# kausaltech/reina-model

Measured on NVIDIA B200. Metric: agent-days/sec (HUS 1.7M), higher is better.
Workload: dtype int32/f32 state, f64 uniforms

## Files before the change

### include/reina_b200.h

```cpp
#ifndef REINA_B200_H
#define REINA_B200_H

#include <stdint.h>

#ifdef __cplusplus
extern "C" {
#endif

#define RB_MAX_AGES 128
#define RB_MAX_VARIANTS 4
#define RB_MAX_ROWS 96
#define RB_NCDF 100
#define RB_MAX_IMPORT_EVENTS 8
#define RB_MAX_VACC 8
#define RB_MAX_IMPORT_CLASSES 16
#define RB_N_PLACES 6
#define RB_IOT_LEN 21

enum { RB_ASYMPTOMATIC = 0, RB_MILD, RB_SEVERE, RB_CRITICAL, RB_FATAL };
enum { RB_SUSCEPTIBLE = 0, RB_INCUBATION, RB_ILLNESS, RB_HOSPITALIZED, RB_IN_ICU, RB_RECOVERED, RB_DEAD };
enum { RB_NO_PROBLEMOS = 0, RB_TOO_MANY_INFECTEES, RB_TOO_MANY_CONTACTS, RB_HOSPITAL_ACCOUNTING_FAILURE,
       RB_NEGATIVE_CONTACTS, RB_MALLOC_FAILURE, RB_OTHER_FAILURE, RB_WRONG_STATE,
       RB_CONTACT_PROBABILITY_FAILURE, RB_INFECTEES_MISMATCH };
enum { RB_NO_TESTING = 0, RB_ALL_WITH_SYMPTOMS_CT, RB_ALL_WITH_SYMPTOMS, RB_ONLY_SEVERE_SYMPTOMS };
// ... 72 lines not shown
int rb_create(const rb_config *cfg, const int32_t *age_counts, const int32_t *group_of_age,
              const rb_variant *variants, const int32_t *import_lo, const int32_t *import_hi,
              const float *import_cum, rb_engine **out);
void rb_destroy(rb_engine *e);

int rb_reset(rb_engine *e, uint32_t seed);

int rb_set_initial_state(rb_engine *e, const int32_t *ipc7);

int rb_set_contact_table(rb_engine *e, int32_t epoch, const int32_t *n_rows, const double *cum_p,
                         const int32_t *age_lo, const int32_t *age_hi, const uint8_t *place,
                         const float *mask_p, const double *nr_contacts, const double *ncontact_cdf);

int rb_set_schedule(rb_engine *e, int32_t day0, int32_t n, const rb_day_params *params);

int rb_step(rb_engine *e, int32_t n_days);
int rb_sync(rb_engine *e);
int32_t rb_day(rb_engine *e);

int rb_snapshot(rb_engine *e);
int32_t rb_row_len(rb_engine *e);
int rb_read_stats(rb_engine *e, int32_t day0, int32_t n, int32_t *out);

int rb_read_moments(rb_engine *e, int32_t day0, int32_t n, double *sum, double *sumsq);

int rb_read_per_age(rb_engine *e, int32_t replica, int32_t attr, int32_t *out);

int rb_problem(rb_engine *e, int32_t *out);

int rb_sample(rb_engine *e, int32_t what, int32_t age, int32_t severity, int32_t n, int32_t *out);

int rb_rng_block(int32_t words, uint32_t key, const uint32_t *ctr, uint32_t *out);

int rb_read_agents(rb_engine *e, int32_t replica, rb_agent *out);
int rb_read_queue(rb_engine *e, int32_t replica, int32_t *out, int32_t cap, int32_t *n);
int rb_read_available(rb_engine *e, int32_t replica, int32_t *beds_icu);
float rb_last_step_ms(rb_engine *e);
#define RB_N_KERNELS 5
int rb_step_profiled(rb_engine *e, int32_t n_days, float *ms_per_kernel);
int rb_step_timed(rb_engine *e, int32_t n_days, float *ms_per_kernel, int32_t *launches_per_kernel, float *wall_ms);
int rb_comm_init(rb_engine *e, int32_t rank, int32_t nranks, const uint8_t *unique_id128);
int32_t rb_comm_rank(rb_engine *e);
int32_t rb_comm_size(rb_engine *e);
int rb_comm_allreduce(rb_engine *e, double *inout, int64_t n, int32_t op);
int rb_comm_allgather(rb_engine *e, const void *in, void *out, int64_t bytes_per_rank);
int rb_reduce_moments(rb_engine *e, int32_t day0, int32_t n, double *sum, double *sumsq, int64_t *n_replicas);

int rb_shard_unique_id(uint8_t *out128);
int rb_shard_init(rb_engine *e, int32_t rank, int32_t nranks, const uint8_t *unique_id128, float exchange_capacity);
int rb_shard_init_local(rb_engine **engines, int32_t nranks, float exchange_capacity);
int32_t rb_shard_rank(rb_engine *e);
int32_t rb_shard_nranks(rb_engine *e);
int64_t rb_shard_message_bytes(rb_engine *e);
int32_t rb_shard_exchange(rb_engine *e);

int64_t rb_state_bytes(rb_engine *e);
int rb_save_state(rb_engine *e, void *out, int64_t capacity);
int rb_load_state(rb_engine *e, const void *in, int64_t n_bytes);

void rb_debug_flag(rb_engine *e, int32_t flag);
int rb_debug_phase_cycles(rb_engine *e, int32_t replica, long long *out16);

int64_t rb_launch_count(rb_engine *e);
int64_t rb_copied_bytes(rb_engine *e, int32_t direction);
const char *rb_last_error(void);

// ... 5 lines not shown
```

### reina_b200/_abi.py

```python
import ctypes as C
import os

import numpy as np

RB_MAX_AGES = 128
RB_MAX_VARIANTS = 4
RB_MAX_ROWS = 96
RB_NCDF = 100
RB_MAX_IMPORT_EVENTS = 8
RB_MAX_VACC = 8
RB_MAX_IMPORT_CLASSES = 16
RB_N_PLACES = 6
RB_IOT_LEN = 21
RB_N_TABLES = 6

ATTRS = ['susceptible', 'vaccinated', 'infected', 'all_infected', 'detected', 'all_detected',
         'in_icu', 'cum_icu', 'in_ward', 'dead', 'recovered', 'non_hospital_deaths', 'new_infections']
RB_N_ATTRS = len(ATTRS)
SCALARS = ['available_icu_units', 'available_hospital_beds', 'total_icu_units', 'total_hospital_beds',
           'total_infections', 'total_infectors', 'exposed_per_day', 'ct_cases_per_day', 'table_epoch',
           'day']
RB_S_CONTACTS0 = len(SCALARS)
RB_S_VARIANT0 = RB_S_CONTACTS0 + RB_N_PLACES
RB_N_SCALARS = RB_S_VARIANT0 + RB_MAX_VARIANTS
# ... 27 lines not shown


class DayParams(C.Structure):
    _fields_ = [
        ('testing_mode', C.c_int32), ('p_detected_anyway', C.c_float),
        ('p_successful_tracing', C.c_float), ('beds_delta', C.c_int32), ('icu_delta', C.c_int32),
        ('table_epoch', C.c_int32), ('n_imports', C.c_int32),
        ('import_amount', C.c_int32 * RB_MAX_IMPORT_EVENTS),
        ('import_variant', C.c_int32 * RB_MAX_IMPORT_EVENTS),
        ('trickle', C.c_int32 * RB_MAX_VARIANTS), ('n_vacc', C.c_int32),
        ('vacc_nr', C.c_int32 * RB_MAX_VACC), ('vacc_min_age', C.c_int32 * RB_MAX_VACC),
        ('vacc_max_age', C.c_int32 * RB_MAX_VACC), ('vacc_slot', C.c_int32 * RB_MAX_VACC),
        ('import_traced', C.c_int32), ('reserved', C.c_int32 * 3),
    ]


AGENT_DTYPE = np.dtype([
    ('infector', '<i4'), ('n_infected', '<i4'), ('days_left', '<i2'), ('day_of_illness', '<i2'),
    ('day_of_vaccination', '<i2'), ('state', 'u1'), ('severity', 'u1'), ('variant', 'u1'),
    ('flags', 'u1'), ('ward_days', 'u1'), ('icu_days', 'u1')], align=True)
assert AGENT_DTYPE.itemsize == 20, AGENT_DTYPE.itemsize

_HERE = os.path.dirname(os.path.abspath(__file__))
CUDA_LIB_PATH = os.environ.get('REINA_B200_LIB') or os.path.join(_HERE, 'libreina_b200.so')

SYMBOLS = ['create', 'destroy', 'reset', 'set_initial_state', 'step_profiled', 'set_contact_table', 'set_schedule', 'step', 'sync', 'day',
           'snapshot', 'row_len', 'read_stats', 'read_moments', 'read_per_age', 'problem', 'sample', 'read_agents',
           'read_queue', 'read_available', 'last_step_ms', 'launch_count', 'last_error', 'rng_block']


SHARD_SYMBOLS = ['shard_unique_id', 'shard_init', 'shard_init_local', 'shard_rank', 'shard_nranks', 'shard_message_bytes', 'shard_exchange',
                 'state_bytes', 'save_state', 'load_state',
                 'comm_init', 'comm_rank', 'comm_size', 'comm_allreduce', 'comm_allgather', 'reduce_moments',
                 'step_timed', 'debug_flag', 'debug_phase_cycles', 'copied_bytes']
SH_SHIFT = 12


def owner_of(agent_index, nranks):
    return (np.asarray(agent_index) >> SH_SHIFT) % nranks


class EngineError(RuntimeError):
    pass


def _ptr(a, ctype):
    return a.ctypes.data_as(C.POINTER(ctype))


class Library:

    def __init__(self, path, prefix):
        if not os.path.exists(path):
            raise EngineError(
                '%s not found: build it with `python -c "import __graft_entry__ as g; g.build()"` '
                '(there is no CPU fallback)' % path)
        self.path, self.prefix = path, prefix
        self.dll = C.CDLL(path)
        f = {}
        for name in SYMBOLS:
            f[name] = getattr(self.dll, prefix + name)
        vp = C.c_void_p
        f['create'].argtypes = [C.POINTER(Config), C.POINTER(C.c_int32), C.POINTER(C.c_int32),
                                C.POINTER(Variant), C.POINTER(C.c_int32), C.POINTER(C.c_int32),
                                C.POINTER(C.c_float), C.POINTER(vp)]
        f['destroy'].argtypes = [vp]
        f['destroy'].restype = None
# ... 24 lines not shown
        f['last_step_ms'].argtypes = [vp]
        f['last_step_ms'].restype = C.c_float
        f['launch_count'].argtypes = [vp]
        f['launch_count'].restype = C.c_int64
        f['last_error'].argtypes = []
        f['last_error'].restype = C.c_char_p
        if prefix == 'rb_':
            for name in SHARD_SYMBOLS:
                f[name] = getattr(self.dll, prefix + name)
            f['shard_unique_id'].argtypes = [C.c_char_p]
            f['shard_init'].argtypes = [vp, C.c_int32, C.c_int32, C.c_char_p, C.c_float]
            f['shard_init_local'].argtypes = [C.POINTER(vp), C.c_int32, C.c_float]
            f['shard_rank'].argtypes = [vp]
            f['shard_nranks'].argtypes = [vp]
            f['shard_message_bytes'].argtypes = [vp]
            f['shard_message_bytes'].restype = C.c_int64
            f['shard_exchange'].argtypes = [vp]
            f['state_bytes'].argtypes = [vp]
            f['state_bytes'].restype = C.c_int64
            f['save_state'].argtypes = [vp, C.c_void_p, C.c_int64]
            f['load_state'].argtypes = [vp, C.c_void_p, C.c_int64]
            f['comm_init'].argtypes = [vp, C.c_int32, C.c_int32, C.c_char_p]
            f['comm_rank'].argtypes = [vp]
            f['comm_size'].argtypes = [vp]
            f['comm_allreduce'].argtypes = [vp, C.POINTER(C.c_double), C.c_int64, C.c_int32]
            f['comm_allgather'].argtypes = [vp, C.c_void_p, C.c_void_p, C.c_int64]
            f['reduce_moments'].argtypes = [vp, C.c_int32, C.c_int32, C.POINTER(C.c_double), C.POINTER(C.c_double), C.POINTER(C.c_int64)]
            f['step_timed'].argtypes = [vp, C.c_int32, C.POINTER(C.c_float), C.POINTER(C.c_int32), C.POINTER(C.c_float)]
            f['debug_flag'].argtypes = [vp, C.c_int32]
            f['debug_flag'].restype = None
            f['debug_phase_cycles'].argtypes = [vp, C.c_int32, C.c_void_p]
            f['copied_bytes'].argtypes = [vp, C.c_int32]
            f['copied_bytes'].restype = C.c_int64
        self.f = f

    def check(self, rc, what):
        if rc != 0:
            raise EngineError('%s%s failed (%d): %s' % (
                self.prefix, what, rc, (self.f['last_error']() or b'').decode(errors='replace')))


_cuda_lib = None


def cuda_library():
    global _cuda_lib
    if _cuda_lib is None:
        _cuda_lib = Library(CUDA_LIB_PATH, 'rb_')
    return _cuda_lib


class Engine:

    def __init__(self, lib, cfg, age_counts, group_of_age, variants, import_lo, import_hi, import_cum):
        self.lib = lib
        self.cfg = cfg
        self.n_agents, self.n_ages = cfg.n_agents, cfg.n_ages
        self.n_groups, self.n_replicas = cfg.n_groups, cfg.n_replicas
        age_counts = np.ascontiguousarray(age_counts, dtype=np.int32)
        group_of_age = np.ascontiguousarray(group_of_age, dtype=np.int32)
        import_lo = np.ascontiguousarray(import_lo, dtype=np.int32)
        import_hi = np.ascontiguousarray(import_hi, dtype=np.int32)
        import_cum = np.ascontiguousarray(import_cum, dtype=np.float32)
        varr = (Variant * len(variants))(*variants)
        h = C.c_void_p()
        lib.check(lib.f['create'](C.byref(cfg), _ptr(age_counts, C.c_int32), _ptr(group_of_age, C.c_int32),
# ... 183 lines not shown
```

### reina_b200/csrc/engine.cu

```cuda
#include "state.cuh"
#include "boundary.cuh"
#include "sweep.cuh"
#include "contacts.cuh"
#include "shard.cuh"
#include "setup.cuh"
#include "run.cuh"

static thread_local char g_err[512];
#define CK(call) do { cudaError_t e_ = (call); if (e_ != cudaSuccess) { snprintf(g_err, sizeof g_err, "%s:%d %s: %s", __FILE__, __LINE__, #call, cudaGetErrorString(e_)); return 1; } } while (0)

#define MAX_GROUPS 8
struct ReplicaGroup {
    int r0, R;
    int sweep_blocks, list_blocks, resolve_blocks;
    cudaStream_t stream;
    cudaEvent_t ev_stagger, ev_join;
    cudaGraphExec_t graph[2];
};

struct rb_engine {
    rb_config cfg;
    Eng G;
    cudaStream_t stream;
    cudaEvent_t ev0, ev1;
    std::vector<void *> allocs;
    std::vector<DevTable *> tables;
    std::vector<std::vector<uint8_t>> table_args, table_host;
    DevTable **d_tables;
    int n_table_slots;
    rb_day_params *d_sched;
    double *d_moments;
    void *h_stage; int n_stage;
    cudaEvent_t ev_stage[4];
    std::vector<rb_day_params> h_sched;
    std::vector<int32_t> age_start, age_counts;
    std::vector<rb_variant> h_variants;
    int32_t day;
    float last_ms;
    int64_t launches;
    int64_t h2d_bytes, d2h_bytes;
    int sweep_blocks, list_blocks, resolve_blocks;
    cudaGraphExec_t graph[2];
    bool have_graphs;
    cudaError_t launch_err;
// ... 146 lines not shown
    float cc = cfg->contact_capacity > 0 ? cfg->contact_capacity : 1.0f;
    G.cap_items = pow2_at_least((uint64_t)((double)N * cc) + 4096);
    G.cap_succ = pow2_at_least((uint64_t)N / 8 + 4096);
    G.cap_events = pow2_at_least((uint64_t)N / 16 + 2048);
    G.cap_queue = pow2_at_least((uint64_t)N / 8 + 2048);
    const size_t RN = (size_t)R * G.Npad;
    cudaDeviceProp prop; CK(cudaGetDeviceProperties(&prop, cfg->device));
    const int sms = prop.multiProcessorCount;
    e->run_ctas = 0; e->run_boundary_ctas = 1;
    {
        int per_sm = 0;
        CK(cudaOccupancyMaxActiveBlocksPerMultiprocessor(&per_sm, k_run, RUN_THREADS, 0));
        const long long total = (long long)per_sm * sms;
        bool on = false;
        if (const char *s = getenv("RB_PERSISTENT")) on = atoi(s) != 0;
        if (on && total >= 2LL * R) {
            long long t = total / R; if (t > 64) t = 64;
            if (const char *s = getenv("RB_RUN_CTAS")) { const int v = atoi(s); if (v >= 1 && (long long)v * R <= total) t = v; }
            e->run_ctas = (int)t;
            int b = 1; while (b * 2 <= t && b * 2 <= 16) b *= 2;
            e->run_boundary_ctas = b;
        }
    }
    {
        int ng, pct;
        group_config(R, &ng, &pct);
        long long ctas = (long long)sms * SW_CTAS_PER_SM * (ng > 1 ? pct : 100) / 100 / ((R + ng - 1) / ng);
        if (ctas < 1) ctas = 1;
        long long S = 2 * ctas * SW_WARPS, most = (long long)N / 256;
        if (e->run_ctas) S = 2LL * e->run_ctas * RUN_WARPS;
        if (S > most) S = most;
        G.n_seg = (uint32_t)(S < 1 ? 1 : S);
        G.seg_cap = ((uint32_t)N + G.n_seg - 1) / G.n_seg;
    }
    G.sus_words = ((G.Npad + 31) / 32 + 32 + 3) & ~3;
    if (dalloc(e, &G.hot, RN) || dalloc(e, &G.perm, RN) || dalloc(e, &G.rec, RN) ||
        dalloc(e, &G.sus, (size_t)R * G.sus_words) || dalloc(e, &G.det, (size_t)R * G.sus_words) || dalloc(e, &G.alist, (size_t)R * 2 * G.n_seg * G.seg_cap) || dalloc(e, &G.seg_n, (size_t)R * 2 * G.n_seg) || dalloc(e, &G.items, (size_t)R * G.cap_items) || dalloc(e, &G.succ, (size_t)R * G.cap_succ) ||
        dalloc(e, &G.ev_key, (size_t)R * G.cap_events) || dalloc(e, &G.ev_agent, (size_t)R * G.cap_events) ||
        dalloc(e, &G.q_key, (size_t)R * 2 * G.cap_queue) || dalloc(e, &G.q_agent, (size_t)R * 2 * G.cap_queue) ||
        dalloc(e, &G.ctr, (size_t)R) || dalloc(e, &G.stats, (size_t)R * (cfg->max_days + 1) * G.row_len) ||
        dalloc(e, &e->d_sched, (size_t)cfg->max_days + 1) ||
        dalloc(e, &e->d_moments, 2 * ((size_t)cfg->max_days + 1) * G.row_len + 2)) { rb_destroy(e); return 1; }
    G.sched = e->d_sched;
    e->h_sched.assign(cfg->max_days + 1, rb_day_params());
    e->n_table_slots = 1024;
    if (dalloc(e, &e->d_tables, (size_t)e->n_table_slots)) { rb_destroy(e); return 1; }
    CK(cudaMemset(e->d_tables, 0, sizeof(DevTable *) * e->n_table_slots));
    G.tables = e->d_tables;
    e->tables.assign(e->n_table_slots, nullptr);
    rb_variant *dv; int32_t *d_as, *d_ga, *d_ilo, *d_ihi; float *d_icum; uint8_t *d_ab;
    if (dalloc(e, &dv, (size_t)cfg->n_variants) || dalloc(e, &d_as, (size_t)cfg->n_ages + 1) || dalloc(e, &d_ga, (size_t)cfg->n_ages) ||
        dalloc(e, &d_ilo, (size_t)RB_MAX_IMPORT_CLASSES) || dalloc(e, &d_ihi, (size_t)RB_MAX_IMPORT_CLASSES) ||
        dalloc(e, &d_icum, (size_t)RB_MAX_IMPORT_CLASSES) || dalloc(e, &d_ab, (size_t)(G.Npad >> 10) + 2)) { rb_destroy(e); return 1; }
    {
        std::vector<uint8_t> ab((size_t)(G.Npad >> 10) + 2);
        int age = 0;
        for (size_t b = 0; b < ab.size(); b++) {
            int64_t a = (int64_t)b << 10; if (a > N - 1) a = N - 1;
            while (age < cfg->n_ages - 1 && e->age_start[age + 1] <= a) age++;
            ab[b] = (uint8_t)age;
        }
        CK(cudaMemcpy(d_ab, ab.data(), ab.size(), cudaMemcpyHostToDevice));
    }
    e->h_variants.assign(variants, variants + cfg->n_variants);
    CK(cudaMemcpy(dv, variants, sizeof(rb_variant) * cfg->n_variants, cudaMemcpyHostToDevice));
    CK(cudaMemcpy(d_as, e->age_start.data(), sizeof(int32_t) * (cfg->n_ages + 1), cudaMemcpyHostToDevice));
    CK(cudaMemcpy(d_ga, group_of_age, sizeof(int32_t) * cfg->n_ages, cudaMemcpyHostToDevice));
    CK(cudaMemcpy(d_ilo, import_lo, sizeof(int32_t) * cfg->n_import_classes, cudaMemcpyHostToDevice));
    CK(cudaMemcpy(d_ihi, import_hi, sizeof(int32_t) * cfg->n_import_classes, cudaMemcpyHostToDevice));
    CK(cudaMemcpy(d_icum, import_cum, sizeof(float) * cfg->n_import_classes, cudaMemcpyHostToDevice));
    G.age_blk = d_ab; G.variants = dv; G.age_start = d_as; G.group_of_age = d_ga; G.import_lo = d_ilo; G.import_hi = d_ihi; G.import_cum = d_icum;
    e->age_counts.assign(age_counts, age_counts + cfg->n_ages);
    CK(cudaMemset(G.stats, 0, sizeof(int32_t) * (size_t)R * (cfg->max_days + 1) * G.row_len));
    CK(cudaMemset(e->d_sched, 0, sizeof(rb_day_params) * ((size_t)cfg->max_days + 1)));
    int want = ((int)G.n_seg + SW_WARPS - 1) / SW_WARPS;
// ... 690 lines not shown
    e->day += n_days;
    return 0;
}

extern "C" int rb_sync(rb_engine *e) {
    CK(cudaSetDevice(e->cfg.device));
    CK(cudaStreamSynchronize(e->stream));
    float ms = 0;
    if (cudaEventElapsedTime(&ms, e->ev0, e->ev1) == cudaSuccess) e->last_ms = ms; else cudaGetLastError();
    if (!e->shard_events.empty()) {
        double t[6] = {0, 0, 0, 0, 0, 0};
        for (size_t d = 0; d + 7 <= e->shard_events.size(); d += 7)
            for (int k = 0; k < 6; k++) { float x = 0; if (cudaEventElapsedTime(&x, e->shard_events[d + k], e->shard_events[d + k + 1]) == cudaSuccess) t[k] += x; }
        fprintf(stderr, "[rank %d] %zu days: sweep %.2f  expose %.2f  exchange+wait %.2f  merge %.2f  resolve %.2f  boundary %.2f ms (step %.2f)\n",
                e->G.rank, e->shard_events.size() / 7, t[0], t[1], t[2], t[3], t[4], t[5], e->last_ms);
        for (cudaEvent_t ev : e->shard_events) cudaEventDestroy(ev);
        e->shard_events.clear();
    }
    return 0;
}

extern "C" int32_t rb_day(rb_engine *e) { return e->day; }
extern "C" void rb_debug_flag(rb_engine *e, int32_t v) { e->G.dbg = v; }
extern "C" int rb_debug_phase_cycles(rb_engine *e, int32_t replica, long long *out16) {
    cudaSetDevice(e->cfg.device); cudaStreamSynchronize(e->stream);
    RepCtr c; if (cudaMemcpy(&c, &e->G.ctr[replica], sizeof c, cudaMemcpyDeviceToHost) != cudaSuccess) return 1;
    memcpy(out16, c.dbg_t, sizeof c.dbg_t); return 0;
}
extern "C" int rb_rng_block(int32_t words, uint32_t key, const uint32_t *ctr, uint32_t *out) {
    if (words == 4) { const u32x4 x = philox(key, ctr[0], ctr[1], ctr[2], ctr[3]); out[0] = x.x; out[1] = x.y; out[2] = x.z; out[3] = x.w; return 0; }
    snprintf(g_err, sizeof g_err, "rb_rng_block: words must be 4");
    return 1;
}
extern "C" int32_t rb_row_len(rb_engine *e) { return e->G.row_len; }
extern "C" float rb_last_step_ms(rb_engine *e) { return e->last_ms; }
extern "C" int64_t rb_launch_count(rb_engine *e) { return e->launches; }
extern "C" int64_t rb_copied_bytes(rb_engine *e, int32_t direction) { return direction == 0 ? e->h2d_bytes : e->d2h_bytes; }

extern "C" int rb_snapshot(rb_engine *e) {
    CK(cudaSetDevice(e->cfg.device));
    k_snapshot<<<e->G.R, 256, 0, e->stream>>>(e->G); e->launches++;
    CK(cudaGetLastError());
    return 0;
}

extern "C" int rb_read_stats(rb_engine *e, int32_t day0, int32_t n, int32_t *out) {
    CK(cudaSetDevice(e->cfg.device));
    if (day0 < 0 || day0 + n > e->cfg.max_days + 1) { snprintf(g_err, sizeof g_err, "stats range"); return 1; }
    const Eng &G = e->G;
    CK(cudaMemcpy2DAsync(out, sizeof(int32_t) * (size_t)n * G.row_len,
                         G.stats + (size_t)day0 * G.row_len, sizeof(int32_t) * (size_t)(G.max_days + 1) * G.row_len,
                         sizeof(int32_t) * (size_t)n * G.row_len, G.R, cudaMemcpyDeviceToHost, e->stream));
    CK(cudaStreamSynchronize(e->stream));
    e->d2h_bytes += (int64_t)sizeof(int32_t) * n * G.row_len * G.R;
    return 0;
}

extern "C" int rb_read_moments(rb_engine *e, int32_t day0, int32_t n, double *sum, double *sumsq) {
    CK(cudaSetDevice(e->cfg.device));
    if (day0 < 0 || n < 1 || day0 + n > e->cfg.max_days + 1) { snprintf(g_err, sizeof g_err, "stats range"); return 1; }
    const size_t cnt = (size_t)n * e->G.row_len;
    double *d = e->d_moments;
    k_moments<<<n, 160, 0, e->stream>>>(e->G, day0, d, d + cnt); e->launches++;
    CK(cudaGetLastError());
    CK(cudaMemcpyAsync(sum, d, sizeof(double) * cnt, cudaMemcpyDeviceToHost, e->stream));
    CK(cudaMemcpyAsync(sumsq, d + cnt, sizeof(double) * cnt, cudaMemcpyDeviceToHost, e->stream));
// ... 163 lines not shown
```

### reina_b200/csrc/state.cuh

```cuda
#ifndef REINA_B200_STATE_CUH
#define REINA_B200_STATE_CUH

#include <cuda_runtime.h>
#include <stdint.h>
#include <stdio.h>
#include <string.h>

#include <dlfcn.h>
#include <nccl.h>

#include <algorithm>
#include <vector>

#include "../../include/reina_b200.h"
#include "rng.cuh"

#define MAX_INFECTEES 64
#define MAX_CONTACTS 128

#define H_STATE(h) ((h) & 7u)
#define H_SEV(h) (((h) >> 3) & 7u)
#define H_DET (1u << 6)
#define H_QUEUED (1u << 7)
#define H_VAR(h) (((h) >> 8) & 3u)
#define H_FRESH (1u << 10)
#define H_INCL (1u << 11)
#define H_LIST (1u << 12)
#define H_VACC (1u << 13)
#define H_DL(h) (((h) >> 14) & 255u)
#define H_DOI(h) (((h) >> 22) & 31u)
#define H_PEND (1u << 27)
#define H_DAYS_MASK ((255u << 14) | (31u << 22))
#define H_SET_STATE(h, s) (((h) & ~7u) | (uint32_t)(s))
#define H_SET_DL(h, d) (((h) & ~(255u << 14)) | ((uint32_t)(d) << 14))
#define H_SET_DOI(h, d) (((h) & ~(31u << 22)) | ((uint32_t)(d) << 22))

#define KEY_IDLE 0xFFFFFFFFFFFFFFFFull
#define QKEY_SWEEP (1ull << 62)
#define CT_DEAD (1ull << 61)
#define CT_DECIDED (1ull << 60)
#define CT_KEYMASK ((1ull << 60) - 1ull)

enum { EV_HOSP_CLAIM = 0, EV_WARD_RELEASE = 1, EV_TO_ICU = 2, EV_ICU_RELEASE = 3 };

#define MAX_RANKS 16
#define WIDE_MAX_CTAS 64
#define SORT_SMEM 2048
#ifndef PRE_THREADS
#define PRE_THREADS 512
#endif
#define NEG_INF (-(1 << 29))

#ifndef GUIDE_BITS
#define GUIDE_BITS 12
#endif
struct DevTable {
    int32_t n_rows[RB_MAX_AGES];
    float nr_contacts[RB_MAX_AGES];
    double ncdf[RB_MAX_AGES][2][RB_NCDF];
    double cum_p[RB_MAX_AGES][RB_MAX_ROWS];
    uint32_t cum24[RB_MAX_AGES][RB_MAX_ROWS];
    int32_t start[RB_MAX_AGES][RB_MAX_ROWS];
    int32_t size[RB_MAX_AGES][RB_MAX_ROWS];
    float mask_p[RB_MAX_AGES][RB_MAX_ROWS];
    uint8_t place[RB_MAX_AGES][RB_MAX_ROWS];
// ... 34 lines not shown
    alignas(128) uint32_t n_succ;
    alignas(128) int32_t exposed_per_day;
    int32_t total_infectors, total_infections;
    alignas(128) uint32_t n_events;
    uint32_t n_newq;
    uint32_t n_upd;
    alignas(128) int32_t daily_contacts[RB_N_PLACES];
    int32_t by_variant[RB_MAX_VARIANTS];
    alignas(128) int32_t drain_det[RB_MAX_AGES];
    alignas(128) uint32_t n_l0;
    uint32_t n_l1, n_edges;
    alignas(128) unsigned int run_bar;
    unsigned int run_exit;
    alignas(128) unsigned int wide_bar;
    alignas(128) uint32_t wide_day;
    int32_t wide_mp[WIDE_MAX_CTAS][4];
    long long dbg_t[16];
    long long dbg_last;
};

struct Eng {
    int32_t dbg;
    int32_t N, Npad, n_ages, n_groups, n_variants, R, max_days, row_len, n_import_classes, fhalf;
    uint32_t cap_items, cap_succ, cap_events, cap_queue;
    uint32_t *hot;
    uint32_t *perm;
    AgentRec *rec;
    uint32_t *sus;
    int32_t sus_words;
    uint32_t *det;
    uint2 *alist;
    uint2 *seg_n;
    uint32_t n_seg, seg_cap;
    uint2 *items;
    Attempt *succ;
    unsigned long long *ev_key; int32_t *ev_agent;
    unsigned long long *q_key; int32_t *q_agent;
    RepCtr *ctr;
    int32_t *stats;
    const rb_day_params *sched;
    DevTable *const *tables;
    const rb_variant *variants;
    const int32_t *age_start;
    const uint8_t *age_blk;
    const int32_t *group_of_age;
    const int32_t *import_lo, *import_hi; const float *import_cum;
    int32_t rank, nranks;
    int32_t wide_min;
    int32_t r0;
    uint8_t *xbuf; size_t xslot;
    uint8_t *xpeer[MAX_RANKS];
    int32_t xp2p; const uint32_t *xepoch;
    uint32_t xcap_q, xcap_ev, xcap_upd, xcap_succ;
};

#define XFLAG_BYTES 256
#define SH_SHIFT 12
__device__ __forceinline__ uint32_t xflag_value(const Eng &G, int day) { return *G.xepoch * 65536u + (uint32_t)day + 1u; }
__device__ __forceinline__ bool owns(const Eng &G, uint32_t a) { return G.nranks == 1 || (int)((a >> SH_SHIFT) % (uint32_t)G.nranks) == G.rank; }

struct XSlot {
    RepCtr *hdr;
    unsigned long long *q_key; int32_t *q_agent;
    unsigned long long *ev_key; int32_t *ev_agent;
    uint2 *upd;
    struct Attempt *succ;
// ... 32 lines not shown
    const uint32_t s = G.perm[(size_t)r * G.Npad + a];
    return s >= c->start ? s - c->start : s + (uint32_t)G.N - c->start;
}
__device__ __forceinline__ void mark_detected(const Eng &G, int r, int32_t a) {
    atomicOr(&G.det[(size_t)r * G.sus_words + (a >> 5)], 1u << (a & 31));
}
__device__ __forceinline__ void count_add(RepCtr *c, int attr, int age, int d) { atomicAdd(&c->counts[attr][age], d); }
__device__ __forceinline__ void set_problem(RepCtr *c, int p) { atomicCAS(&c->problem, 0, p); }

__device__ __forceinline__ int symptom_severity(const rb_variant *v, int age, float val, bool vacc_eff) {
    float vmod = 1.0f;
    if (vacc_eff) vmod = vmod * 0.1f;
    float syc = v->tab[RB_T_SYMPTOMATIC][age];
    if (val >= syc) return RB_ASYMPTOMATIC;
    syc = syc * vmod;
    float dohc = v->tab[RB_T_DEATH_OUTSIDE_HOSPITAL][age];
    if (dohc != 0.0f) {
        if (val < dohc * syc) return RB_FATAL;
        val = (val - dohc) / (1.0f - dohc);
    }
    float sc = v->tab[RB_T_SEVERE][age], cc = v->tab[RB_T_CRITICAL][age], fc = v->tab[RB_T_FATAL][age];
    if (val < ((fc * cc) * sc) * syc) return RB_FATAL;
    if (val < (cc * sc) * syc) return RB_CRITICAL;
    if (val < sc * syc) return RB_SEVERE;
    return RB_MILD;
}

__device__ __forceinline__ uint2 *seg_ptr(const Eng &G, int r, uint32_t which, uint32_t s) {
    return G.alist + (((size_t)r * 2 + which) * G.n_seg + s) * G.seg_cap;
}
__device__ __forceinline__ uint2 *seg_count(const Eng &G, int r, uint32_t which, uint32_t s) {
    return G.seg_n + ((size_t)r * 2 + which) * G.n_seg + s;
}
__device__ __forceinline__ void list_add(const Eng &G, int r, RepCtr *c, uint32_t which, uint32_t a, uint32_t w) {
    const uint32_t s = a % G.n_seg;
    const uint32_t k = atomicAdd(&seg_count(G, r, which, s)->y, 1u);
    if (k < G.seg_cap) seg_ptr(G, r, which, s)[G.seg_cap - 1u - k] = make_uint2(a, w); else set_problem(c, RB_OTHER_FAILURE);
}

__device__ void device_infect(const Eng &G, int r, RepCtr *c, int32_t t, int32_t src, uint32_t src_h, int variant,
                              int slot, bool fresh, int list, bool has_list) {
    const size_t base = (size_t)r * G.Npad;
    const int day = c->day;
    uint32_t old = 0; int32_t prev_child = -1;
    if (src >= 0) {
        old = atomicAdd(&G.rec[base + src].cold, 1u);
        prev_child = atomicExch(&G.rec[base + src].first_child, t);
    }
    const int vd = c->any_vacc ? (int)G.rec[base + t].vacc_day : -1;
    const int age = age_of(G, t);
    const rb_variant *v0 = &G.variants[0];
    const bool vacc_eff = vd >= 0 && (day - vd) > 14;
    int sev = 0, dl = 0;
    if (owns(G, (uint32_t)t)) {
        u32x4 x = philox(c->seed, (uint32_t)t, (uint32_t)day, PU_SEVERITY, 0);
        sev = symptom_severity(v0, age, u01f(x.x), vacc_eff);
        dl = clamp255(round_to_int(gamma_f(c->seed, (uint32_t)t, (uint32_t)day, PU_INCUB, v0->incubation_kappa, v0->incubation_theta)));
    }
    if (src >= 0) {
        variant = (int)H_VAR(src_h);
        G.rec[base + t].infector = src;
        if ((src_h & H_LIST) && (old & 0xffffu) >= MAX_INFECTEES) set_problem(c, RB_TOO_MANY_INFECTEES);
        G.rec[base + t].inf_key = ((uint32_t)day << 8) | (uint32_t)slot;
        G.rec[base + t].next_sib = prev_child;
    }
    uint32_t nh = (vd >= 0 ? H_VACC : 0u) | RB_INCUBATION | ((uint32_t)sev << 3) | ((uint32_t)variant << 8) | ((uint32_t)dl << 14);
// ... 19 lines not shown
```

### reina_b200/csrc/sweep.cuh

```cuda
#ifndef REINA_B200_SWEEP_CUH
#define REINA_B200_SWEEP_CUH
#include "state.cuh"

#ifndef SW_THREADS
#define SW_THREADS 128
#endif
#define SW_WARPS (SW_THREADS / 32)
#define SW_RCAP 64
#ifndef SW_CTAS_PER_SM
#define SW_CTAS_PER_SM 9
#endif

struct WarpRings {
    uint32_t ea[SW_RCAP], ed[SW_RCAP];
    uint32_t ta[SW_RCAP], tw[SW_RCAP];
};

__device__ __forceinline__ uint32_t ring_push(uint32_t *ra, uint32_t *rb, uint32_t tail, bool want, uint32_t x, uint32_t y, int lane) {
    const uint32_t m = __ballot_sync(0xffffffffu, want);
    if (want) { uint32_t p = (tail + __popc(m & ((1u << lane) - 1u))) & (SW_RCAP - 1); ra[p] = x; rb[p] = y; }
    return tail + __popc(m);
}

__device__ __forceinline__ void seg_append(const Eng &G, RepCtr *c, uint2 *out, uint32_t &out_n, bool want, uint32_t a, uint32_t w, int lane) {
// ... 162 lines not shown
            h = hot & ~H_FRESH;
            if (H_STATE(h) < RB_RECOVERED) { uint32_t dl = H_DL(h); if (dl > 0) dl--; h = H_SET_DL(h, dl); }
        } else h = (hot & ~(H_DAYS_MASK | H_FRESH)) | (w & H_DAYS_MASK);
        const uint32_t st = H_STATE(h);
        if (st >= RB_RECOVERED) {
            removed = true;
            infected_others = (int)(G.rec[base + a].cold & 0xffffu);
            G.hot[base + a] = hot | H_INCL;
        } else if (H_DL(h) == 0) {
            h = transition(G, r, c, O, (int32_t)a, h, lw);
            G.hot[base + a] = h;
            keep = true; changed = true;
        } else { lw = h; keep = true; }
    }
    const uint32_t rm = __ballot_sync(0xffffffffu, removed);
    if (rm) {
#pragma unroll
        for (int o = 16; o > 0; o >>= 1) infected_others += __shfl_xor_sync(0xffffffffu, infected_others, o);
        if (lane == 0) { atomicAdd(&cd->total_infectors, __popc(rm)); if (infected_others) atomicAdd(&cd->total_infections, infected_others); }
    }
    if (keep) list_add(G, r, cd, next, a, lw);
    if (O.upd) {
        const uint32_t mk = __ballot_sync(0xffffffffu, changed);
        uint32_t b = 0;
        if (lane == 0 && mk) b = atomicAdd(&O.cd->n_upd, (uint32_t)__popc(mk));
        b = __shfl_sync(0xffffffffu, b, 0);
        if (changed) {
            const uint32_t idx = b + __popc(mk & ((1u << lane) - 1u));
            if (idx < O.cap_upd) O.upd[idx] = make_uint2(a, h); else set_problem(O.cd, RB_OTHER_FAILURE);
        }
    }
}

__device__ __forceinline__ void stage_entry(const Eng &G, uint32_t &w, bool &keep, bool &want_e, bool &want_t, uint32_t &desc) {
    const uint32_t st = H_STATE(w);
    if ((w & H_PEND) || st >= RB_RECOVERED) { want_t = true; return; }
    if (w & H_FRESH) { w &= ~H_FRESH; keep = true; return; }
    const uint32_t sev = H_SEV(w), var = H_VAR(w);
    uint32_t dl = H_DL(w);
    if (st == RB_INCUBATION || st == RB_ILLNESS) {
        const int dayidx = st == RB_INCUBATION ? -(int)dl : (int)H_DOI(w);
        if (!(w & H_DET) && dayidx >= -10 && dayidx <= 10 && G.variants[var].iot[dayidx + 10] != 0.0f) {
            want_e = true;
            const uint32_t cls = (st == RB_ILLNESS && sev != RB_ASYMPTOMATIC) ? 1u : 0u;
            desc = ((uint32_t)(dayidx + 10) << 14) | ((sev == RB_ASYMPTOMATIC ? 1u : 0u) << 19) | (var << 20) | (cls << 22);
        }
        if (st == RB_ILLNESS) { uint32_t doi = H_DOI(w); if (doi < 31) doi++; w = H_SET_DOI(w, doi); }
    }
    if (dl > 0) dl--;
    w = H_SET_DL(w, dl);
    if (dl == 0) want_t = true; else keep = true;
}

__device__ __forceinline__ void sweep_warp(const Eng &G, const int r, const uint32_t first, const uint32_t n_warps, WarpRings &W, const int lane) {
    RepCtr *c = &G.ctr[r];
    const DevTable *tb = G.tables[c->epoch];
    uint2 *items = G.items + (size_t)r * G.cap_items;
    RepCtr *cd = !G.xbuf ? c : xslot_of(G, G.rank, c->day).hdr;
    const uint32_t cur = c->lsel;
    uint32_t e_head = 0, e_tail = 0, t_head = 0, t_tail = 0;

    uint2 cnt_next = make_uint2(0u, 0u);
    if (first < G.n_seg) cnt_next = *seg_count(G, r, cur, first);
    for (uint32_t seg = first; ; seg += n_warps) {
        const bool tail = seg >= G.n_seg;
        const uint2 cnt = cnt_next;
        cnt_next = make_uint2(0u, 0u);
        if (seg + n_warps < G.n_seg) cnt_next = *seg_count(G, r, cur, seg + n_warps);
        const uint32_t nf = min(cnt.x, G.seg_cap), n = min(cnt.x + cnt.y, G.seg_cap);
        const uint2 *in = seg_ptr(G, r, cur, tail ? 0u : seg);
        uint2 *out = seg_ptr(G, r, cur ^ 1u, tail ? 0u : seg);
        uint32_t out_n = 0;
        const uint32_t gap = G.seg_cap - n;
        auto entry = [&](uint32_t i) { return __ldcs(&in[i < nf ? i : i + gap]); };
        uint2 ent = make_uint2(0u, 0u);
        if ((uint32_t)lane < n) ent = entry(lane);
        uint32_t i0 = 0;
        bool again;
        do {
            if (i0 < n) {
                const bool valid = i0 + lane < n;
                const uint2 cur_ent = ent;
                if (i0 + 32 + lane < n) ent = entry(i0 + 32 + lane);
                bool keep = false, want_e = false, want_t = false;
                uint32_t w = cur_ent.y, desc = 0;
                if (valid) stage_entry(G, w, keep, want_e, want_t, desc);
                seg_append(G, cd, out, out_n, keep, cur_ent.x, w, lane);
                e_tail = ring_push(W.ea, W.ed, e_tail, want_e, cur_ent.x, desc, lane);
                t_tail = ring_push(W.ta, W.tw, t_tail, want_t, cur_ent.x, w, lane);
                __syncwarp();
            }
            const uint32_t e_av = e_tail - e_head, t_av = t_tail - t_head;
            if (e_av >= 32 || (tail && e_av)) { const uint32_t m = min(32u, e_av); stage_expose(G, r, c, cd, tb, W, e_head, m, items, lane); e_head += m; }
            if (t_av >= 32 || (tail && t_av)) { const uint32_t m = min(32u, t_av); stage_slow(G, r, c, cd, W, t_head, m, cur ^ 1u, lane); t_head += m; }
            __syncwarp();
            i0 += 32;
            again = tail ? (e_tail != e_head || t_tail != t_head) : i0 < n;
        } while (again);
        if (tail) break;
        if (lane == 0) seg_count(G, r, cur ^ 1u, seg)->x = out_n;
    }
}
__global__ void __launch_bounds__(SW_THREADS, SW_CTAS_PER_SM) k_sweep(Eng G) {
    __shared__ WarpRings s_rings[SW_WARPS];
    const int warp = threadIdx.x >> 5;
    sweep_warp(G, blockIdx.y + G.r0, blockIdx.x * SW_WARPS + warp, gridDim.x * SW_WARPS, s_rings[warp], threadIdx.x & 31);
}

__global__ void k_flush_lists(Eng G) {
    const int r = blockIdx.y;
    const RepCtr *c = &G.ctr[r];
    const size_t base = (size_t)r * G.Npad;
    const uint32_t cur = c->lsel;
    const int lane = threadIdx.x & 31;
    const uint32_t n_warps = gridDim.x * (blockDim.x >> 5);
    for (uint32_t seg = blockIdx.x * (blockDim.x >> 5) + (threadIdx.x >> 5); seg < G.n_seg; seg += n_warps) {
        const uint2 cnt = *seg_count(G, r, cur, seg);
        const uint32_t nf = min(cnt.x, G.seg_cap), n = min(cnt.x + cnt.y, G.seg_cap);
        const uint2 *in = seg_ptr(G, r, cur, seg);
        for (uint32_t i = lane; i < n; i += 32) {
            const uint2 e = in[i < nf ? i : i + (G.seg_cap - n)];
            if ((e.y & H_PEND) || H_STATE(e.y) >= RB_RECOVERED) continue;
            const uint32_t h = G.hot[base + e.x];
            G.hot[base + e.x] = (h & ~(H_DAYS_MASK | H_FRESH)) | (e.y & (H_DAYS_MASK | H_FRESH));
        }
    }
}
__global__ void k_rebuild_lists(Eng G) {
    const int r = blockIdx.y;
    RepCtr *c = &G.ctr[r];
    const size_t base = (size_t)r * G.Npad;
    const uint32_t cur = c->lsel;
    for (int a = blockIdx.x * blockDim.x + threadIdx.x; a < G.N; a += gridDim.x * blockDim.x) {
        if (!owns(G, (uint32_t)a)) continue;
        uint32_t h = G.hot[base + a];
        const uint32_t st = H_STATE(h);
        if (!((st >= RB_INCUBATION && st <= RB_IN_ICU) || (st >= RB_RECOVERED && !(h & H_INCL)))) continue;
        if (h & H_QUEUED) h |= H_DET;
        G.perm[base + a] = sweep_slot(G, c, (uint32_t)a);
        list_add(G, r, c, cur, (uint32_t)a, h);
    }
}
__global__ void k_clear_lists(Eng G) {
    const size_t n = (size_t)G.R * 2 * G.n_seg;
    for (size_t i = (size_t)blockIdx.x * blockDim.x + threadIdx.x; i < n; i += (size_t)gridDim.x * blockDim.x) G.seg_n[i] = make_uint2(0u, 0u);
}

#endif
```

Before: 743.9 billion.

## Park quiet active agents in phased buckets to skip daily sweep work

Adds per-segment 'park' buckets, K phases by default, that hold active agents whose next several days are provably uneventful. The daily sweep reads only today's bucket, catches each parked entry up by the days elapsed using a 4-bit day tag, and so avoids rereading and rewriting every quiet agent each day. Flush and clear kernels now handle the park buckets, and a host self-check compares park_advance against repeated stage_entry calls. The cost is extra memory, warp ballot and shuffle work per parked batch, and a risk of overflow or state drift if the quiet-day predicate is wrong.

```diff
diff --git a/include/reina_b200.h b/include/reina_b200.h
--- a/include/reina_b200.h
+++ b/include/reina_b200.h
@@ -128,6 +128,8 @@
 
 int rb_rng_block(int32_t words, uint32_t key, const uint32_t *ctr, uint32_t *out);
 
+int64_t rb_park_check(void);
+
 int rb_read_agents(rb_engine *e, int32_t replica, rb_agent *out);
 int rb_read_queue(rb_engine *e, int32_t replica, int32_t *out, int32_t cap, int32_t *n);
 int rb_read_available(rb_engine *e, int32_t replica, int32_t *beds_icu);
diff --git a/reina_b200/_abi.py b/reina_b200/_abi.py
--- a/reina_b200/_abi.py
+++ b/reina_b200/_abi.py
@@ -83,7 +83,7 @@
 SHARD_SYMBOLS = ['shard_unique_id', 'shard_init', 'shard_init_local', 'shard_rank', 'shard_nranks', 'shard_message_bytes', 'shard_exchange',
                  'state_bytes', 'save_state', 'load_state',
                  'comm_init', 'comm_rank', 'comm_size', 'comm_allreduce', 'comm_allgather', 'reduce_moments',
-                 'step_timed', 'debug_flag', 'debug_phase_cycles', 'copied_bytes']
+                 'step_timed', 'debug_flag', 'debug_phase_cycles', 'copied_bytes', 'park_check']
 SH_SHIFT = 12
 
 
@@ -174,6 +174,8 @@
             f['debug_phase_cycles'].argtypes = [vp, C.c_int32, C.c_void_p]
             f['copied_bytes'].argtypes = [vp, C.c_int32]
             f['copied_bytes'].restype = C.c_int64
+            f['park_check'].argtypes = []
+            f['park_check'].restype = C.c_int64
         self.f = f
 
     def check(self, rc, what):
diff --git a/reina_b200/csrc/engine.cu b/reina_b200/csrc/engine.cu
--- a/reina_b200/csrc/engine.cu
+++ b/reina_b200/csrc/engine.cu
@@ -10,6 +10,9 @@
 #define CK(call) do { cudaError_t e_ = (call); if (e_ != cudaSuccess) { snprintf(g_err, sizeof g_err, "%s:%d %s: %s", __FILE__, __LINE__, #call, cudaGetErrorString(e_)); return 1; } } while (0)
 
 #define MAX_GROUPS 8
+#ifndef PARK_K_DEFAULT
+#define PARK_K_DEFAULT 4
+#endif
 struct ReplicaGroup {
     int r0, R;
     int sweep_blocks, list_blocks, resolve_blocks;
@@ -222,6 +225,9 @@
         if (S > most) S = most;
         G.n_seg = (uint32_t)(S < 1 ? 1 : S);
         G.seg_cap = ((uint32_t)N + G.n_seg - 1) / G.n_seg;
+        int k = PARK_K_DEFAULT;
+        if (const char *s = getenv("RB_PARK")) k = atoi(s);
+        G.park_k = (uint32_t)(k < 2 ? 0 : (k > 16 ? 16 : k));
     }
     G.sus_words = ((G.Npad + 31) / 32 + 32 + 3) & ~3;
     if (dalloc(e, &G.hot, RN) || dalloc(e, &G.perm, RN) || dalloc(e, &G.rec, RN) ||
@@ -231,6 +237,7 @@
         dalloc(e, &G.ctr, (size_t)R) || dalloc(e, &G.stats, (size_t)R * (cfg->max_days + 1) * G.row_len) ||
         dalloc(e, &e->d_sched, (size_t)cfg->max_days + 1) ||
         dalloc(e, &e->d_moments, 2 * ((size_t)cfg->max_days + 1) * G.row_len + 2)) { rb_destroy(e); return 1; }
+    if (G.park_k && (dalloc(e, &G.park, (size_t)R * G.n_seg * G.park_k * G.seg_cap) || dalloc(e, &G.park_n, (size_t)R * G.n_seg * G.park_k))) { rb_destroy(e); return 1; }
     G.sched = e->d_sched;
     e->h_sched.assign(cfg->max_days + 1, rb_day_params());
     e->n_table_slots = 1024;
@@ -987,6 +994,28 @@
     snprintf(g_err, sizeof g_err, "rb_rng_block: words must be 4");
     return 1;
 }
+extern "C" int64_t rb_park_check(void) {
+    rb_variant v; memset(&v, 0, sizeof v);
+    for (int i = 0; i < RB_IOT_LEN; i++) v.iot[i] = 1.0f;
+    Eng G; memset(&G, 0, sizeof G);
+    G.variants = &v;
+    int64_t bad = 0;
+    for (uint32_t st = RB_INCUBATION; st <= RB_IN_ICU; st++)
+        for (uint32_t sev = RB_ASYMPTOMATIC; sev <= RB_MILD; sev++)
+            for (uint32_t det = 0; det < 2; det++)
+                for (uint32_t dl = 0; dl < 256; dl++)
+                    for (uint32_t doi = 0; doi < 32; doi++) {
+                        const uint32_t w0 = st | (sev << 3) | (det ? H_DET : 0u) | (dl << 14) | (doi << 22);
+                        const uint32_t q = park_quiet_days(w0);
+                        uint32_t w = w0;
+                        for (uint32_t j = 1; j <= q; j++) {
+                            bool keep = false, want_e = false, want_t = false; uint32_t desc = 0;
+                            stage_entry(G, w, keep, want_e, want_t, desc);
+                            if (!keep || want_e || want_t || w != park_advance(w0 | ((j & 15u) << 28), j)) { bad++; break; }
+                        }
+                    }
+    return bad;
+}
 extern "C" int32_t rb_row_len(rb_engine *e) { return e->G.row_len; }
 extern "C" float rb_last_step_ms(rb_engine *e) { return e->last_ms; }
 extern "C" int64_t rb_launch_count(rb_engine *e) { return e->launches; }
diff --git a/reina_b200/csrc/state.cuh b/reina_b200/csrc/state.cuh
--- a/reina_b200/csrc/state.cuh
+++ b/reina_b200/csrc/state.cuh
@@ -31,6 +31,8 @@
 #define H_DOI(h) (((h) >> 22) & 31u)
 #define H_PEND (1u << 27)
 #define H_DAYS_MASK ((255u << 14) | (31u << 22))
+#define H_TAG(h) ((h) >> 28)
+#define H_TAG_MASK (15u << 28)
 #define H_SET_STATE(h, s) (((h) & ~7u) | (uint32_t)(s))
 #define H_SET_DL(h, d) (((h) & ~(255u << 14)) | ((uint32_t)(d) << 14))
 #define H_SET_DOI(h, d) (((h) & ~(31u << 22)) | ((uint32_t)(d) << 22))
@@ -131,6 +133,9 @@
     uint2 *alist;
     uint2 *seg_n;
     uint32_t n_seg, seg_cap;
+    uint2 *park;
+    uint32_t *park_n;
+    uint32_t park_k;
     uint2 *items;
     Attempt *succ;
     unsigned long long *ev_key; int32_t *ev_agent;
@@ -229,6 +234,27 @@
 __device__ __forceinline__ uint2 *seg_count(const Eng &G, int r, uint32_t which, uint32_t s) {
     return G.seg_n + ((size_t)r * 2 + which) * G.n_seg + s;
 }
+__device__ __forceinline__ uint2 *park_ptr(const Eng &G, int r, uint32_t s, uint32_t k) {
+    return G.park + (((size_t)r * G.n_seg + s) * G.park_k + k) * G.seg_cap;
+}
+__device__ __forceinline__ uint32_t *park_count(const Eng &G, int r, uint32_t s) {
+    return G.park_n + ((size_t)r * G.n_seg + s) * G.park_k;
+}
+__host__ __device__ __forceinline__ uint32_t park_quiet_days(uint32_t w) {
+    const uint32_t st = H_STATE(w), dl = H_DL(w);
+    uint32_t q = dl > 1u ? dl - 1u : 0u;
+    if (!(w & H_DET)) {
+        if (st == RB_INCUBATION) { const uint32_t e = dl > 10u ? dl - 10u : 0u; if (e < q) q = e; }
+        else if (st == RB_ILLNESS && H_DOI(w) <= 10u) q = 0;
+    }
+    return q;
+}
+__host__ __device__ __forceinline__ uint32_t park_advance(uint32_t w, uint32_t e) {
+    w = H_SET_DL(w & ~H_TAG_MASK, H_DL(w) - e);
+    if (H_STATE(w) == RB_ILLNESS) { const uint32_t doi = H_DOI(w) + e; w = H_SET_DOI(w, doi < 31u ? doi : 31u); }
+    return w;
+}
+
 __device__ __forceinline__ void list_add(const Eng &G, int r, RepCtr *c, uint32_t which, uint32_t a, uint32_t w) {
     const uint32_t s = a % G.n_seg;
     const uint32_t k = atomicAdd(&seg_count(G, r, which, s)->y, 1u);
diff --git a/reina_b200/csrc/sweep.cuh b/reina_b200/csrc/sweep.cuh
--- a/reina_b200/csrc/sweep.cuh
+++ b/reina_b200/csrc/sweep.cuh
@@ -218,7 +218,7 @@
     }
 }
 
-__device__ __forceinline__ void stage_entry(const Eng &G, uint32_t &w, bool &keep, bool &want_e, bool &want_t, uint32_t &desc) {
+__host__ __device__ __forceinline__ void stage_entry(const Eng &G, uint32_t &w, bool &keep, bool &want_e, bool &want_t, uint32_t &desc) {
     const uint32_t st = H_STATE(w);
     if ((w & H_PEND) || st >= RB_RECOVERED) { want_t = true; return; }
     if (w & H_FRESH) { w &= ~H_FRESH; keep = true; return; }
@@ -244,34 +244,61 @@
     uint2 *items = G.items + (size_t)r * G.cap_items;
     RepCtr *cd = !G.xbuf ? c : xslot_of(G, G.rank, c->day).hdr;
     const uint32_t cur = c->lsel;
+    const uint32_t K = G.park_k, day = (uint32_t)c->day;
+    const uint32_t ph_today = K ? day % K : 0u;
     uint32_t e_head = 0, e_tail = 0, t_head = 0, t_tail = 0;
 
     uint2 cnt_next = make_uint2(0u, 0u);
-    if (first < G.n_seg) cnt_next = *seg_count(G, r, cur, first);
+    uint32_t pc_next = 0;
+    if (first < G.n_seg) { cnt_next = *seg_count(G, r, cur, first); if ((uint32_t)lane < K) pc_next = park_count(G, r, first)[lane]; }
     for (uint32_t seg = first; ; seg += n_warps) {
         const bool tail = seg >= G.n_seg;
         const uint2 cnt = cnt_next;
-        cnt_next = make_uint2(0u, 0u);
-        if (seg + n_warps < G.n_seg) cnt_next = *seg_count(G, r, cur, seg + n_warps);
+        uint32_t pc = pc_next;
+        cnt_next = make_uint2(0u, 0u); pc_next = 0;
+        if (seg + n_warps < G.n_seg) { cnt_next = *seg_count(G, r, cur, seg + n_warps); if ((uint32_t)lane < K) pc_next = park_count(G, r, seg + n_warps)[lane]; }
         const uint32_t nf = min(cnt.x, G.seg_cap), n = min(cnt.x + cnt.y, G.seg_cap);
+        const uint32_t np = min(__shfl_sync(0xffffffffu, pc, ph_today), G.seg_cap);
+        if ((uint32_t)lane == ph_today) pc = 0;
+        const uint32_t nt = n + np;
         const uint2 *in = seg_ptr(G, r, cur, tail ? 0u : seg);
         uint2 *out = seg_ptr(G, r, cur ^ 1u, tail ? 0u : seg);
         uint32_t out_n = 0;
         const uint32_t gap = G.seg_cap - n;
-        auto entry = [&](uint32_t i) { return __ldcs(&in[i < nf ? i : i + gap]); };
+        auto entry = [&](uint32_t i) { return i < n ? __ldcs(&in[i < nf ? i : i + gap]) : __ldcs(&park_ptr(G, r, seg, ph_today)[i - n]); };
         uint2 ent = make_uint2(0u, 0u);
-        if ((uint32_t)lane < n) ent = entry(lane);
+        if ((uint32_t)lane < nt) ent = entry(lane);
         uint32_t i0 = 0;
         bool again;
         do {
-            if (i0 < n) {
-                const bool valid = i0 + lane < n;
+            if (i0 < nt) {
+                const bool valid = i0 + lane < nt;
                 const uint2 cur_ent = ent;
-                if (i0 + 32 + lane < n) ent = entry(i0 + 32 + lane);
+                if (i0 + 32 + lane < nt) ent = entry(i0 + 32 + lane);
                 bool keep = false, want_e = false, want_t = false;
                 uint32_t w = cur_ent.y, desc = 0;
+                if (valid && i0 + lane >= n) w = park_advance(w, (day - H_TAG(w)) & 15u);
                 if (valid) stage_entry(G, w, keep, want_e, want_t, desc);
+                bool park = false;
+                uint32_t ph = 0;
+                if (keep && K) {
+                    const uint32_t q = park_quiet_days(w);
+                    if (q) {
+                        park = true; keep = false;
+                        ph = ph_today + 1u + min(q, K - 2u); if (ph >= K) ph -= K;
+                        w |= ((day + 1u) & 15u) << 28;
+                    }
+                }
                 seg_append(G, cd, out, out_n, keep, cur_ent.x, w, lane);
+                for (uint32_t pm = __ballot_sync(0xffffffffu, park); pm; ) {
+                    const uint32_t lph = __shfl_sync(0xffffffffu, ph, __ffs(pm) - 1);
+                    const bool mine = park && ph == lph;
+                    const uint32_t m = __ballot_sync(0xffffffffu, mine);
+                    const uint32_t p = __shfl_sync(0xffffffffu, pc, lph) + __popc(m & ((1u << lane) - 1u));
+                    if (mine) { if (p < G.seg_cap) park_ptr(G, r, seg, lph)[p] = make_uint2(cur_ent.x, w); else set_problem(cd, RB_OTHER_FAILURE); }
+                    if ((uint32_t)lane == lph) pc += __popc(m);
+                    pm &= ~m;
+                }
                 e_tail = ring_push(W.ea, W.ed, e_tail, want_e, cur_ent.x, desc, lane);
                 t_tail = ring_push(W.ta, W.tw, t_tail, want_t, cur_ent.x, w, lane);
                 __syncwarp();
@@ -281,10 +308,11 @@
             if (t_av >= 32 || (tail && t_av)) { const uint32_t m = min(32u, t_av); stage_slow(G, r, c, cd, W, t_head, m, cur ^ 1u, lane); t_head += m; }
             __syncwarp();
             i0 += 32;
-            again = tail ? (e_tail != e_head || t_tail != t_head) : i0 < n;
+            again = tail ? (e_tail != e_head || t_tail != t_head) : i0 < nt;
         } while (again);
         if (tail) break;
         if (lane == 0) seg_count(G, r, cur ^ 1u, seg)->x = out_n;
+        if ((uint32_t)lane < K) park_count(G, r, seg)[lane] = pc;
     }
 }
 __global__ void __launch_bounds__(SW_THREADS, SW_CTAS_PER_SM) k_sweep(Eng G) {
@@ -310,6 +338,16 @@
             const uint32_t h = G.hot[base + e.x];
             G.hot[base + e.x] = (h & ~(H_DAYS_MASK | H_FRESH)) | (e.y & (H_DAYS_MASK | H_FRESH));
         }
+        for (uint32_t k = 0; k < G.park_k; k++) {
+            const uint32_t np = min(park_count(G, r, seg)[k], G.seg_cap);
+            const uint2 *pin = park_ptr(G, r, seg, k);
+            for (uint32_t i = lane; i < np; i += 32) {
+                const uint2 e = pin[i];
+                const uint32_t w = park_advance(e.y, ((uint32_t)c->day - H_TAG(e.y)) & 15u);
+                const uint32_t h = G.hot[base + e.x];
+                G.hot[base + e.x] = (h & ~(H_DAYS_MASK | H_FRESH)) | (w & H_DAYS_MASK);
+            }
+        }
     }
 }
 __global__ void k_rebuild_lists(Eng G) {
@@ -328,8 +366,9 @@
     }
 }
 __global__ void k_clear_lists(Eng G) {
-    const size_t n = (size_t)G.R * 2 * G.n_seg;
+    const size_t n = (size_t)G.R * 2 * G.n_seg, np = (size_t)G.R * G.n_seg * G.park_k;
     for (size_t i = (size_t)blockIdx.x * blockDim.x + threadIdx.x; i < n; i += (size_t)gridDim.x * blockDim.x) G.seg_n[i] = make_uint2(0u, 0u);
+    for (size_t i = (size_t)blockIdx.x * blockDim.x + threadIdx.x; i < np; i += (size_t)gridDim.x * blockDim.x) G.park_n[i] = 0u;
 }
 
 #endif
```

Measured after the change: 748.5 billion, median of 6. About the same (+0.6%).
